# afermg/aliby

Measured on AMD Instinct MI355X. Metric: FOV tiles/sec (whole node), higher is better.
Workload: dtype u16 pixels, f64 feature accumulators, f32 dynamics, bfloat16 U-Net

## Files before the change

### aliby_amd/csrc/nn_conv.hip

```cpp
#include "common.h"
#include <utility>

typedef __bf16 bf16x8_t __attribute__((ext_vector_type(8)));
typedef float f32x16_t __attribute__((ext_vector_type(16)));
typedef float f32x2_t __attribute__((ext_vector_type(2)));

namespace {

template <class F, int... I>
__device__ __forceinline__ void static_for_impl(F&& f, std::integer_sequence<int, I...>) {
  (f(std::integral_constant<int, I>{}), ...);
}
template <int N, class F>
__device__ __forceinline__ void static_for(F&& f) {
  static_for_impl(static_cast<F&&>(f), std::make_integer_sequence<int, N>{});
}

__device__ __forceinline__ float cv_bf2f(unsigned h) { return __uint_as_float(h << 16); }
typedef __bf16 bf16x2_t __attribute__((ext_vector_type(2)));
__device__ __forceinline__ unsigned cv_pack2(float lo, float hi) {
  const f32x2_t f = {lo, hi};
  const bf16x2_t b = __builtin_convertvector(f, bf16x2_t);
  return __builtin_bit_cast(unsigned, b);
}
// ... 311 lines not shown
          const bool ok = lx != gapi && c >= 0 && c < a.W && !(bp == TW && kb == TW) && (unsigned)gy < (unsigned)a.H;
          const int img = (snd && ok) ? g0 + 1 : g0;
          inside |= (unsigned)ok << u;
          later |= (unsigned)snd << u;
          if constexpr (C3_HACK & 1) v[u] = make_uint4(cy, c, img, 3);
          else v[u] = inN[(unsigned)(((img * a.H + cy) * IW + min(max(c, 0), a.W - 1)) * a.cs + pl)];
        } else {
          const int gxi = x0 - 1 + lx;
          inside |= (unsigned)((unsigned)gy < (unsigned)a.H && (unsigned)gxi < (unsigned)a.W) << u;
          const int cx = min(max(gxi, 0), a.W - 1);
          if constexpr (C3_HACK & 1) v[u] = make_uint4(cy, cx, 2, 3);
          else v[u] = inN[(unsigned)(((UP ? cy >> 1 : cy) * IW + (UP ? cx >> 1 : cx)) * a.cs + pl)];
        }
      }
#pragma unroll
      for (int u = 0; u < BATCH; ++u) {
        if (it0 + u >= ITERS) break;
        uint4 o;
        if constexpr (PACK) {
          f32x2_t shs[4];
#pragma unroll
          for (int k = 0; k < 4; ++k) shs[k] = ((later >> u) & 1u) ? sh1[k] : sh[k];
          o = conv_act8(v[u], sc, shs, 0u - ((inside >> u) & 1u));
        } else {
          if constexpr (C3_HACK & 16) o = v[u]; else o = conv_act8(v[u], sc, sh, 0u - ((inside >> u) & 1u));
        }
        if (it0 + u == ITERS - 1 && p0 + (it0 + u) * PIX_PER_IT >= RAW) continue;
        if constexpr (C3_HACK & 32) { if (o.x == 0x12345u) lds[pl * PLANE + p0 + (it0 + u) * PIX_PER_IT] = o; }
        else lds[pl * PLANE + p0 + (it0 + u) * PIX_PER_IT] = o;
      }
    }
    if constexpr (PK > 0) {
      constexpr int POCT = 2 * PK, PUNITS = TH * TW * POCT;
      const uint4* pN = a.pin + (size_t)n * a.H * a.W * a.pcs;
#pragma unroll
      for (int it = 0; it < (PUNITS + 255) / 256; ++it) {
        const int u = tid + it * 256;
        if (u >= PUNITS) break;
        const int oct = u % POCT, pix = u / POCT;
        const int cy = min(y0 + pix / TW, a.H - 1), cx = min(x0 + pix % TW, a.W - 1);
        uint4 v = make_uint4(0, 0, 0, 0);
        if (oct < a.pcs) v = pN[(unsigned)((cy * a.W + cx) * a.pcs + oct)];
        ldsP[oct * PPLANE + pix] = v;
      }
    }
    CONV_STAMP(3);
    if constexpr (!(C3_HACK & 128)) __syncthreads();
    CONV_STAMP(4);

#pragma unroll
    for (int pass = 0; pass < PASSES; ++pass) {
      const int rbase = (rg * PASSES + pass) * R;
      f32x16_t acc[R];
      {
        float4 b4[4];
#pragma unroll
        for (int q = 0; q < 4; ++q) b4[q] = (C3_HACK & 64) ? make_float4(0.f, 0.f, 0.f, 0.f) : sbias[(c0 >> 2) + q];
        conv_seed<R>(acc, b4, rr, a.res != nullptr && !(C3_HACK & 2));
      }
      __builtin_amdgcn_sched_barrier(0);
      if (pass + 1 < PASSES && a.res && !(C3_HACK & 2)) load_res(pass + 1);
      __builtin_amdgcn_sched_barrier(0);
      if constexpr (!(C3_HACK & 8))
      conv_mfma<R, KC, (POOL ? cfg::DEPTH_POOL : cfg::DEPTH), PLANE, LW>(
          reinterpret_cast<const bf16x8_t*>(lds) + hh * PLANE + rbase * LW + px + second, wfrag, acc);
      if constexpr (PK > 0) {
        const bf16x8_t* LP = reinterpret_cast<const bf16x8_t*>(ldsP) + hh * PPLANE + rbase * TW + px;
#pragma unroll
        for (int r = 0; r < R; ++r)
#pragma unroll
          for (int k = 0; k < PK; ++k)
            acc[r] = __builtin_amdgcn_mfma_f32_32x32x16_bf16(pfrag[k], LP[2 * k * PPLANE + r * TW], acc[r], 0, 0, 0);
      }
      if (pass == PASSES - 1) CONV_STAMP(5);
      if constexpr (HEAD) {
        __builtin_amdgcn_sched_barrier(0);
#pragma unroll
        for (int r = 0; r < R; ++r) {
          const f32x16_t y = head_from_acc(acc[r], hconst, hconst + 32, hwf, hh);
          const int gy = y0 + rbase + r;
          if (hh == 0 && gx < a.W && gy < a.H) {
            float* hp = a.hout + (size_t)n * a.hO * a.H * a.W + (size_t)gy * a.W + gx;
            const float yo[4] = {y[0], y[1], y[2], y[3]};
            for (int o = 0; o < a.hO; ++o) hp[(size_t)o * a.H * a.W] = yo[o] + hconst[64 + o];
          }
        }
      }
      if ((!HEAD || a.out) && (!(C3_HACK & 4) || acc[0][3] == 12345.f)) conv_store<R>(a, nimg, irow, y0 + rbase, gx, c0, acc);
      if constexpr (POOL) {
        const int PH = a.H >> 1, PW = a.W >> 1;
#pragma unroll
        for (int r = 0; r < R; r += 2) {
          const int gy = y0 + rbase + r;
          const bool writer = (px & 1) == 0 && gx + 1 < a.W && gy + 1 < a.H;
          uint4* pp = a.pool + (size_t)nimg * PH * PW * a.ocs + a.ocoff + (unsigned)((((irow + gy) >> 1) * PW + (gx >> 1)) * a.ocs + (c0 >> 3));
#pragma unroll
          for (int half = 0; half < 2; ++half) {
            unsigned pk[4];
#pragma unroll
            for (int q = 0; q < 4; ++q) {
              const float v0 = fmaxf(acc[r][half * 8 + 2 * q], acc[r + 1][half * 8 + 2 * q]);
              const float v1 = fmaxf(acc[r][half * 8 + 2 * q + 1], acc[r + 1][half * 8 + 2 * q + 1]);
              pk[q] = cv_pack2(fmaxf(v0, __shfl_xor(v0, 1)), fmaxf(v1, __shfl_xor(v1, 1)));
            }
            if (writer) pp[half] = make_uint4(pk[0], pk[1], pk[2], pk[3]);
          }
        }
      }
    }
    CONV_STAMP(6);
  }
}

template <int CIN, int COUT, bool UP, bool PACK = false>
struct DmaCfg {
  static constexpr int KC = CIN / 16, NPL = CIN / 8, NCB = COUT / 32;
  static constexpr int WAVES_PER_SIMD = CIN >= 128 ? 1 : 2;
  static constexpr int R = CIN >= 64 ? 2 : 4;
  static constexpr int PASSES = (CIN >= 128 || COUT >= 128) ? 2 : 1;
  static constexpr int RG = 4 / NCB;
  static constexpr int TH = RG * R * PASSES, TW = 32, LH = TH + 2, LW = TW + 2 + (PACK ? 1 : 0);
  static constexpr int RAW = LH * LW;
  static constexpr int PLANE = NPL == 4 ? RAW + (10 - RAW % 8) % 8 : (RAW | 1);
  static constexpr int A_SLOTS = NPL * PLANE;
  static constexpr int PIX_PER_IT = 256 / NPL;
  static constexpr int ITERS = (RAW + PIX_PER_IT - 1) / PIX_PER_IT;
  static constexpr int RLH = UP ? TH / 2 + 2 : LH, RLW = UP ? TW / 2 + 2 : LW;
  static constexpr int RUNITS = RLH * RLW * NPL;
  static constexpr int GIT = (RUNITS + 255) / 256;
  static constexpr int R_SLOTS = GIT * 256;
  static constexpr int LDS_BYTES = (A_SLOTS + R_SLOTS) * 16;
  static constexpr int DEPTH = (CIN >= 64 && COUT >= 64) ? 4 : 6;
};

template <int CIN, int COUT, bool UP, bool PACK = false>
__global__ __launch_bounds__(256, (DmaCfg<CIN, COUT, UP, PACK>::WAVES_PER_SIMD)) void k_conv3x3_dma(ConvArgs a) {
  static_assert(!PACK || UP, "the packed LDS-DMA variant is written for upsampled input");
  using cfg = DmaCfg<CIN, COUT, UP, PACK>;
  constexpr int KC = cfg::KC, NPL = cfg::NPL, NCB = cfg::NCB, R = cfg::R, TH = cfg::TH, TW = cfg::TW;
  constexpr int LW = cfg::LW, RAW = cfg::RAW, PLANE = cfg::PLANE, RLW = cfg::RLW, PASSES = cfg::PASSES;
  constexpr int PIX_PER_IT = cfg::PIX_PER_IT, ITERS = cfg::ITERS, GIT = cfg::GIT;
  extern __shared__ uint4 lds[];
  uint4* const ldsA = lds;
  uint4* const ldsR = lds + cfg::A_SLOTS;

  const int tid = threadIdx.x, lane = tid & 63, wave = tid >> 6;
  const int cb = wave % NCB, rg = wave / NCB;
  const int px = lane & 31, hh = lane >> 5;
  const int c0 = cb * 32 + hh * 16;

  bf16x8_t wfrag[9 * KC];
  {
    const bf16x8_t* wp = reinterpret_cast<const bf16x8_t*>(a.wpk) + (size_t)cb * 9 * KC * 64 + lane;
#pragma unroll
    for (int i = 0; i < 9 * KC; ++i) wfrag[i] = wp[i * 64];
  }
  const int pl = tid % NPL, pix0 = tid / NPL;
  const int ly0 = pix0 / LW, lx0 = pix0 - ly0 * LW;
  f32x2_t sc[4];
#pragma unroll
  for (int k = 0; k < 4; ++k) sc[k] = f32x2_t{a.scale[pl * 8 + 2 * k], a.scale[pl * 8 + 2 * k + 1]};

  const int IH = UP ? a.H >> 1 : a.H, IW = UP ? a.W >> 1 : a.W;
  const int xcd = blockIdx.x & 7, slot = blockIdx.x >> 3, nslots = gridDim.x >> 3;
  const int per_xcd = (a.ntiles + 7) >> 3;
  const int t_end = min(a.ntiles, (xcd + 1) * per_xcd);
  const int wave_u = __builtin_amdgcn_readfirstlane(wave);

  auto issue_dma = [&](int tile) {
    const int tx = tile % a.tiles_x, tyn = tile / a.tiles_x;
    const int ty = tyn % a.tiles_y, n = tyn / a.tiles_y;
    const int ry0 = UP ? (ty * TH >> 1) - 1 : ty * TH - 1, rx0 = UP ? (tx * TW >> 1) - 1 : tx * TW - 1;
    int g0 = 0, cst = 0, half = 1 << 20;
    if constexpr (PACK) {
      g0 = (tx * TW) / a.W;
      cst = tx * TW - g0 * a.W;
      half = (a.W - cst) >> 1;
    }
    const uint4* inN = a.in + (size_t)(PACK ? n * a.G : n) * IH * IW * a.cs + a.coff;
    int t0 = tid;
    asm volatile("" : "+v"(t0));
#pragma unroll
    for (int k = 0; k < GIT; ++k) {
      const int unit = t0 + k * 256;
      const int rpix = unit / NPL, oct = unit % NPL;
      const int rly = rpix / RLW, rlx = rpix - rly * RLW;
      const int iy = min(max(ry0 + rly, 0), IH - 1);
      int ix, img = 0;
      if constexpr (PACK) {
        const bool first = rlx <= half;
        ix = min(max(first ? (cst >> 1) - 1 + rlx : rlx - half - 1, 0), IW - 1);
        img = first ? g0 : min(g0 + 1, a.G - 1);
      } else {
        ix = min(max(rx0 + rlx, 0), IW - 1);
      }
      const uint4* g = inN + (unsigned)(((img * IH + iy) * IW + ix) * a.cs + oct);
      __builtin_amdgcn_global_load_lds((const __attribute__((address_space(1))) void*)g,
                                       (__attribute__((address_space(3))) void*)(ldsR + k * 256 + wave_u * 64), 16, 0, 0);
    }
  };

  int tile = xcd * per_xcd + slot, stamp_tile = 0;
  if (tile < t_end) issue_dma(tile);
  for (; tile < t_end; tile += nslots, ++stamp_tile) {
    CONV_STAMP(0);
    const int tx = tile % a.tiles_x, tyn = tile / a.tiles_x;
    const int ty = tyn % a.tiles_y, n = tyn / a.tiles_y;
    const int y0 = ty * TH, x0 = tx * TW;
    int g0 = 0, cst = x0, kb = 1 << 20, nimg = n;
    if constexpr (PACK) {
      g0 = x0 / a.W;
      cst = x0 - g0 * a.W;
      kb = a.W - cst;
      nimg = n * a.G;
    }
    const int second = (PACK && px >= kb) ? 1 : 0;
    const int gx = PACK ? (second ? px - kb : cst + px) : x0 + px;
    const int irow = PACK ? (g0 + second) * a.H : 0;

    f32x2_t sh[4], sh1[PACK ? 4 : 1];
    {
      const float* sp = a.shift + (size_t)(nimg + g0) * a.shift_stride + pl * 8;
#pragma unroll
      for (int k = 0; k < 4; ++k) sh[k] = f32x2_t{sp[2 * k], sp[2 * k + 1]};
      if constexpr (PACK) {
        const float* sq = a.shift + (size_t)(nimg + min(g0 + 1, a.G - 1)) * a.shift_stride + pl * 8;
#pragma unroll
        for (int k = 0; k < 4; ++k) sh1[k] = f32x2_t{sq[2 * k], sq[2 * k + 1]};
      }
    }
    float4 b4[4] = {};
    if (a.bias) {
      const float4* bp = reinterpret_cast<const float4*>(a.bias + c0);
#pragma unroll
      for (int q = 0; q < 4; ++q) b4[q] = bp[q];
    }
    uint4 rr[R][2];
    auto load_res = [&](int pass) { conv_load_res<R>(a, nimg, irow, y0 + (rg * PASSES + pass) * R, gx, c0, rr); };
    if (a.res && !(C3_HACK & 2)) load_res(0);
    CONV_STAMP(1);
    asm volatile("s_waitcnt vmcnt(0)" ::: "memory");
    __syncthreads();
    CONV_STAMP(2);
    {
      const int ry0 = UP ? (y0 >> 1) - 1 : y0 - 1, rx0 = UP ? (x0 >> 1) - 1 : x0 - 1;
      int p0 = pix0, qy = ly0, qx = lx0;
      asm volatile("" : "+v"(p0), "+v"(qy), "+v"(qx));
#pragma unroll
      for (int it = 0; it < ITERS; ++it) {
        int lx = qx + (it * PIX_PER_IT) % LW, ly = qy + (it * PIX_PER_IT) / LW;
        if (lx >= LW) { lx -= LW; ly += 1; }
        const int gy = y0 - 1 + ly, gxi = x0 - 1 + lx;
        const int pix = p0 + it * PIX_PER_IT;
        unsigned keep;
        int rpix;
        uint4 o;
        if constexpr (PACK) {
          const int gapi = kb < 32 ? kb + 1 : TW + 2;
          const int bp = lx - 1 - (lx > gapi ? 1 : 0);
          const int snd = bp >= kb ? 1 : 0;
          const int c = snd ? bp - kb : cst + bp;
          keep = 0u - (unsigned)(lx != gapi && c >= 0 && c < a.W && !(bp == TW && kb == TW) && (unsigned)gy < (unsigned)a.H);
          const int rcol = snd ? (kb >> 1) + 1 + (c >> 1) : ((cst + bp) >> 1) - ((cst >> 1) - 1);
          rpix = min(max(((gy >> 1) - ry0) * RLW + rcol, 0), cfg::RLH * RLW - 1);
          f32x2_t shs[4];
#pragma unroll
          for (int k = 0; k < 4; ++k) shs[k] = snd ? sh1[k] : sh[k];
          o = conv_act8(ldsR[rpix * NPL + pl], sc, shs, keep);
        } else {
          keep = 0u - (unsigned)((unsigned)gy < (unsigned)a.H && (unsigned)gxi < (unsigned)a.W);
          rpix = UP ? min(((gy >> 1) - ry0) * RLW + ((gxi >> 1) - rx0), cfg::RLH * RLW - 1) : min(pix, RAW - 1);
          o = conv_act8(ldsR[rpix * NPL + pl], sc, sh, keep);
        }
        if (it == ITERS - 1 && pix >= RAW) continue;
        ldsA[pl * PLANE + pix] = o;
      }
    }
    CONV_STAMP(3);
    __syncthreads();
#pragma unroll
    for (int pass = 0; pass < PASSES; ++pass) {
      const int rbase = (rg * PASSES + pass) * R;
      f32x16_t acc[R];
      conv_seed<R>(acc, b4, rr, a.res != nullptr);
      __builtin_amdgcn_sched_barrier(0);
      if (pass == 0 && tile + nslots < t_end) issue_dma(tile + nslots);
      if (pass + 1 < PASSES && a.res) load_res(pass + 1);
      __builtin_amdgcn_sched_barrier(0);
      if (pass == 0) CONV_STAMP(4);
      conv_mfma<R, KC, cfg::DEPTH, PLANE, LW>(reinterpret_cast<const bf16x8_t*>(ldsA) + hh * PLANE + rbase * LW + px + second, wfrag, acc);
      if (pass == PASSES - 1) CONV_STAMP(5);
      conv_store<R>(a, nimg, irow, y0 + rbase, gx, c0, acc);
    }
    CONV_STAMP(6);
  }
}

struct PairCfg {
  static constexpr int KC = 2, NPL = 4, R = 2, PASSES = 2;
  static constexpr int TH = 14, TWO = 30, MH = 16, MW = 32, IH = 18, IW = 34;
  static constexpr int RAW_IN = IH * IW, PLANE_IN = RAW_IN + (10 - RAW_IN % 8) % 8;
  static constexpr int RAW_MID = MH * MW, PLANE_MID = RAW_MID + (10 - RAW_MID % 8) % 8;
  static constexpr int PIX_PER_IT = 256 / NPL, ITERS = (RAW_IN + PIX_PER_IT - 1) / PIX_PER_IT;
  static constexpr int MID_SLOTS = NPL * PLANE_MID + 8;
  static constexpr int SLOTS = NPL * PLANE_IN + 2 * MID_SLOTS;
  static constexpr int LDS_BYTES = SLOTS * 16;
  static constexpr int DEPTH = 6;
};

#ifndef CP_HACK
#define CP_HACK 0
#endif
template <bool POOL, bool HEAD>
__global__ __launch_bounds__(512, 1) void k_conv_pair32(ConvArgs a) {
  static_assert(!(POOL && HEAD), "either the pooled output (down block) or the output head (last unit)");
  using cfg = PairCfg;
  constexpr int KC = cfg::KC, NPL = cfg::NPL, R = cfg::R, PASSES = cfg::PASSES, TH = cfg::TH, TWO = cfg::TWO;
  constexpr int IW_ = cfg::IW, MW = cfg::MW, PLANE_IN = cfg::PLANE_IN, PLANE_MID = cfg::PLANE_MID, RAW_IN = cfg::RAW_IN;
  constexpr int PIX_PER_IT = cfg::PIX_PER_IT, ITERS = cfg::ITERS;
  extern __shared__ uint4 lds[];
  uint4* const ldsIn = lds;
  uint4* const ldsMid0 = lds + NPL * PLANE_IN;
  __shared__ __align__(16) float tabB[64];
  __shared__ float hconst[HEAD ? 2 * 32 + 4 : 1];

  const int consumer = threadIdx.x >> 8;
  const int tid = threadIdx.x & 255, lane = tid & 63, wave = tid >> 6;
  const int px = lane & 31, hh = lane >> 5;
  const int c0 = hh * 16;

  const int xcd = blockIdx.x & 7, slot = blockIdx.x >> 3, nslots = gridDim.x >> 3;
  const int per_xcd = (a.ntiles + 7) >> 3;
  const int t_begin = xcd * per_xcd + slot, t_end = min(a.ntiles, (xcd + 1) * per_xcd);
  const int my_tiles = t_begin < t_end ? (t_end - t_begin + nslots - 1) / nslots : 0;

  if (!consumer) {
    bf16x8_t wA[9 * KC];
    {
      const bf16x8_t* pa = reinterpret_cast<const bf16x8_t*>(a.wpk) + lane;
#pragma unroll
      for (int i = 0; i < 9 * KC; ++i) wA[i] = pa[i * 64];
    }
    const int pl = tid % NPL, pix0 = tid / NPL;
    const int ly0 = pix0 / IW_, lx0 = pix0 - ly0 * IW_;
    f32x2_t sc[4];
#pragma unroll
    for (int k = 0; k < 4; ++k) sc[k] = f32x2_t{a.scale[pl * 8 + 2 * k], a.scale[pl * 8 + 2 * k + 1]};
    uint4 v[ITERS];
    unsigned inside = 0;
    auto request = [&](int tile) {
      const int tx = tile % a.tiles_x, tyn = tile / a.tiles_x;
      const int ty = tyn % a.tiles_y, n = tyn / a.tiles_y;
      const int y0 = ty * TH, x0 = tx * TWO;
      const uint4* inN = a.in + (size_t)n * a.H * a.W * a.cs + a.coff;
      inside = 0;
#pragma unroll
      for (int u = 0; u < ITERS; ++u) {
        int lx = lx0 + (u * PIX_PER_IT) % IW_, ly = ly0 + (u * PIX_PER_IT) / IW_;
        if (lx >= IW_) { lx -= IW_; ly += 1; }
        const int gy = y0 - 2 + ly, gxi = x0 - 2 + lx;
        inside |= (unsigned)((unsigned)gy < (unsigned)a.H && (unsigned)gxi < (unsigned)a.W) << u;
        const int cy = min(max(gy, 0), a.H - 1), cx = min(max(gxi, 0), a.W - 1);
        if constexpr (CP_HACK & 1) v[u] = make_uint4(u, 1, 2, 3); else v[u] = inN[(unsigned)((cy * a.W + cx) * a.cs + pl)];
      }
    };
    if (my_tiles > 0) request(t_begin);
    for (int it = 0; it < my_tiles; ++it) {
      const int tile = t_begin + it * nslots;
      const int tx = tile % a.tiles_x, tyn = tile / a.tiles_x;
      const int ty = tyn % a.tiles_y, n = tyn / a.tiles_y;
      const int y0 = ty * TH, x0 = tx * TWO;
      uint4* const ldsMid = ldsMid0 + (it & 1) * cfg::MID_SLOTS;
      f32x2_t sh[4];
      {
        const float* sp = a.shift + (size_t)n * a.shift_stride + pl * 8;
#pragma unroll
        for (int k = 0; k < 4; ++k) sh[k] = f32x2_t{sp[2 * k], sp[2 * k + 1]};
      }
      if (tid < 32) {
        tabB[tid] = a.scale2[tid];
        tabB[32 + tid] = a.shift2[(size_t)n * a.shift2_stride + tid];
      }
#pragma unroll
      for (int u = 0; u < ITERS; ++u) {
        const uint4 o = conv_act8(v[u], sc, sh, 0u - ((inside >> u) & 1u));
        if (u == ITERS - 1 && pix0 + u * PIX_PER_IT >= RAW_IN) continue;
        if constexpr (!(CP_HACK & 64)) ldsIn[pl * PLANE_IN + pix0 + u * PIX_PER_IT] = o;
      }
      __syncthreads();
      if (it + 1 < my_tiles) request(tile + nslots);
      __builtin_amdgcn_sched_barrier(0);
#pragma unroll
      for (int pass = 0; pass < PASSES; ++pass) {
        const int mbase = (wave * PASSES + pass) * R;
        f32x16_t acc[R];
        {
          float4 b4[4] = {};
          if (a.bias) {
            const float4* bp = reinterpret_cast<const float4*>(a.bias + c0);
#pragma unroll
            for (int q = 0; q < 4; ++q) b4[q] = bp[q];
          }
#pragma unroll
          for (int r = 0; r < R; ++r)
#pragma unroll
            for (int q = 0; q < 4; ++q) { acc[r][4 * q] = b4[q].x; acc[r][4 * q + 1] = b4[q].y; acc[r][4 * q + 2] = b4[q].z; acc[r][4 * q + 3] = b4[q].w; }
        }
        __builtin_amdgcn_sched_barrier(0);
        if constexpr (!(CP_HACK & 8)) conv_mfma<R, KC, cfg::DEPTH, PLANE_IN, IW_>(reinterpret_cast<const bf16x8_t*>(ldsIn) + hh * PLANE_IN + mbase * IW_ + px, wA, acc);
        __builtin_amdgcn_sched_barrier(0);
        const int mgx = x0 - 1 + px;
#pragma unroll
        for (int r = 0; r < R; ++r) {
          const int mgy = y0 - 1 + mbase + r;
          const unsigned keep = 0u - (unsigned)((unsigned)mgy < (unsigned)a.H && (unsigned)mgx < (unsigned)a.W);
#pragma unroll
          for (int half = 0; half < 2; ++half) {
            f32x2_t s2[4], h2[4];
            const float4* tp = reinterpret_cast<const float4*>(tabB + c0 + 8 * half);
            const float4 sa = tp[0], sb = tp[1], ha = tp[8], hb = tp[9];
            s2[0] = f32x2_t{sa.x, sa.y}; s2[1] = f32x2_t{sa.z, sa.w}; s2[2] = f32x2_t{sb.x, sb.y}; s2[3] = f32x2_t{sb.z, sb.w};
            h2[0] = f32x2_t{ha.x, ha.y}; h2[1] = f32x2_t{ha.z, ha.w}; h2[2] = f32x2_t{hb.x, hb.y}; h2[3] = f32x2_t{hb.z, hb.w};
            const uint4 raw = make_uint4(cv_pack2(acc[r][8 * half + 0], acc[r][8 * half + 1]), cv_pack2(acc[r][8 * half + 2], acc[r][8 * half + 3]),
                                         cv_pack2(acc[r][8 * half + 4], acc[r][8 * half + 5]), cv_pack2(acc[r][8 * half + 6], acc[r][8 * half + 7]));
            if constexpr (!(CP_HACK & 32)) ldsMid[(2 * hh + half) * PLANE_MID + (mbase + r) * MW + px] = conv_act8(raw, s2, h2, keep);
          }
        }
      }
      __syncthreads();
    }
    __syncthreads();
    __syncthreads();
  } else {
    bf16x8_t wB[9 * KC];
    {
      const bf16x8_t* pb = reinterpret_cast<const bf16x8_t*>(a.wpk2) + lane;
#pragma unroll
      for (int i = 0; i < 9 * KC; ++i) wB[i] = pb[i * 64];
    }
    HeadW hwf;
    if constexpr (HEAD) {
      hwf = head_weights(a.hw, a.hO, lane);
      if (tid < 32) {
        hconst[tid] = a.hscale[tid];
        hconst[32 + tid] = a.hshift[tid];
        if (tid < 4) hconst[64 + tid] = tid < a.hO ? a.hbias[tid] : 0.f;
      }
    }
    float4 b4[4] = {};
    if (a.bias2) {
      const float4* bp = reinterpret_cast<const float4*>(a.bias2 + c0);
#pragma unroll
      for (int q = 0; q < 4; ++q) b4[q] = bp[q];
    }
    __syncthreads();
    __syncthreads();
    for (int it = 0; it < my_tiles; ++it) {
      const int tile = t_begin + it * nslots;
      const int tx = tile % a.tiles_x, tyn = tile / a.tiles_x;
      const int ty = tyn % a.tiles_y, n = tyn / a.tiles_y;
      const int y0 = ty * TH, x0 = tx * TWO;
      const uint4* const ldsMid = ldsMid0 + (it & 1) * cfg::MID_SLOTS;
      const int gx = (px < TWO && x0 + px < a.W) ? x0 + px : a.W;
#pragma unroll
      for (int pass = 0; pass < PASSES; ++pass) {
        const int rbase = (wave * PASSES + pass) * R;
        if (rbase < TH) {
          uint4 rr[R][2];
          if (a.res && !(CP_HACK & 2)) conv_load_res<R>(a, n, 0, y0 + rbase, min(gx, a.W - 1), c0, rr);
          f32x16_t acc[R];
          conv_seed<R>(acc, b4, rr, a.res != nullptr && !(CP_HACK & 2));
          __builtin_amdgcn_sched_barrier(0);
          if constexpr (!(CP_HACK & 16)) conv_mfma<R, KC, cfg::DEPTH, PLANE_MID, MW>(reinterpret_cast<const bf16x8_t*>(ldsMid) + hh * PLANE_MID + rbase * MW + px, wB, acc);
          if constexpr (HEAD) {
#pragma unroll
            for (int r = 0; r < R; ++r) {
              const f32x16_t y = head_from_acc(acc[r], hconst, hconst + 32, hwf, hh);
              const int gy = y0 + rbase + r;
              if (hh == 0 && gx < a.W && gy < a.H) {
                float* hp = a.hout + (size_t)n * a.hO * a.H * a.W + (size_t)gy * a.W + gx;
                const float yo[4] = {y[0], y[1], y[2], y[3]};
                for (int o = 0; o < a.hO; ++o) hp[(size_t)o * a.H * a.W] = yo[o] + hconst[64 + o];
              }
            }
          }
          if ((!HEAD || a.out) && (!(CP_HACK & 4) || acc[0][3] == 12345.f)) conv_store<R>(a, n, 0, y0 + rbase, gx, c0, acc);
          if constexpr (POOL) {
            const int PH = a.H >> 1, PW = a.W >> 1;
            const int gy = y0 + rbase;
            const bool writer = (px & 1) == 0 && gx + 1 < a.W && gy + 1 < a.H;
            uint4* pp = a.pool + (size_t)n * PH * PW * a.ocs + a.ocoff + (unsigned)(((gy >> 1) * PW + (min(gx, a.W - 1) >> 1)) * a.ocs + (c0 >> 3));
#pragma unroll
            for (int half = 0; half < 2; ++half) {
              unsigned pk[4];
#pragma unroll
              for (int q = 0; q < 4; ++q) {
                const float v0 = fmaxf(acc[0][half * 8 + 2 * q], acc[1][half * 8 + 2 * q]);
                const float v1 = fmaxf(acc[0][half * 8 + 2 * q + 1], acc[1][half * 8 + 2 * q + 1]);
                pk[q] = cv_pack2(fmaxf(v0, __shfl_xor(v0, 1)), fmaxf(v1, __shfl_xor(v1, 1)));
              }
              if (writer && (!(CP_HACK & 4) || acc[0][3] == 12345.f)) pp[half] = make_uint4(pk[0], pk[1], pk[2], pk[3]);
            }
          }
        }
        __syncthreads();
      }
    }
  }
}

struct FirstPairCfg {
  static constexpr int KC = 2, NPL = 4, R = 2, PASSES = 2;
  static constexpr int TH = 14, TWO = 30, MH = 16, MW = 32, AH = 18, AW = 36;
  static constexpr int RAW_MID = MH * MW, PLANE_MID = RAW_MID + (10 - RAW_MID % 8) % 8;
  static constexpr int MID_SLOTS = NPL * PLANE_MID + 8;
  static constexpr int P0_WORDS = 2 * AH * AW;
  static constexpr int RAWP_WORDS = MH * MW;
  static constexpr int VALS = 2 * AH * AW, ITERS = (VALS + 255) / 256;
  static constexpr int LDS_BYTES = 2 * MID_SLOTS * 16 + P0_WORDS * 4 + 2 * RAWP_WORDS * 4;
  static constexpr int DEPTH = 6;
};

__global__ __launch_bounds__(512, 1) void k_conv_first_pair(ConvArgs a) {
  using cfg = FirstPairCfg;
  constexpr int KC = cfg::KC, R = cfg::R, PASSES = cfg::PASSES, TH = cfg::TH, TWO = cfg::TWO, MW = cfg::MW;
  constexpr int AH = cfg::AH, AW = cfg::AW, PLANE_MID = cfg::PLANE_MID, ITERS = cfg::ITERS;
  extern __shared__ uint4 lds[];
  uint4* const ldsMid0 = lds;
  unsigned* const P0 = reinterpret_cast<unsigned*>(lds + 2 * cfg::MID_SLOTS);
  unsigned* const rawP0 = P0 + cfg::P0_WORDS;
  __shared__ __align__(16) float tabB[64];

  const int consumer = threadIdx.x >> 8;
  const int tid = threadIdx.x & 255, lane = tid & 63, wave = tid >> 6;
  const int px = lane & 31, hh = lane >> 5;
  const int c0 = hh * 16;

  const int xcd = blockIdx.x & 7, slot = blockIdx.x >> 3, nslots = gridDim.x >> 3;
  const int per_xcd = (a.ntiles + 7) >> 3;
  const int t_begin = xcd * per_xcd + slot, t_end = min(a.ntiles, (xcd + 1) * per_xcd);
  const int my_tiles = t_begin < t_end ? (t_end - t_begin + nslots - 1) / nslots : 0;
  const size_t plane = (size_t)a.H * a.W;

  if (!consumer) {
    bf16x8_t wF[2];
    {
      const int m = lane & 31, co = 16 * ((m >> 2) & 1) + (m & 3) + 4 * (m >> 3);
#pragma unroll
      for (int kc = 0; kc < 2; ++kc) {
        unsigned r4[4];
#pragma unroll
        for (int j2 = 0; j2 < 4; ++j2) {
          float v[2];
#pragma unroll
          for (int e = 0; e < 2; ++e) {
            const int k = 16 * kc + 8 * hh + 2 * j2 + e, c = k / 12, ty = (k % 12) / 4, tx = k % 4;
            v[e] = (c < a.fcin && tx < 3 && k < 24) ? a.fw[((size_t)co * a.fcin + c) * 9 + ty * 3 + tx] : 0.f;
          }
          r4[j2] = cv_pack2(v[0], v[1]);
        }
        wF[kc] = __builtin_bit_cast(bf16x8_t, make_uint4(r4[0], r4[1], r4[2], r4[3]));
      }
    }
    int goff[2][2];
    unsigned gmask[2][2];
#pragma unroll
    for (int kc = 0; kc < 2; ++kc)
#pragma unroll
      for (int g = 0; g < 2; ++g) {
        const int k = 16 * kc + 8 * hh + 4 * g;
        const bool live = k < 24 && k / 12 < a.fcin;
        goff[kc][g] = live ? (k / 12) * AH * AW + ((k % 12) / 4) * AW : 0;
        gmask[kc][g] = live ? 0xffffffffu : 0u;
      }
    if (tid < 32) {
      tabB[tid] = a.scale2[tid];
      tabB[32 + tid] = a.shift2[tid];
    }
    const float fs0 = a.fscale[0], fh0 = a.fshift[0];
    const float fs1 = a.fcin > 1 ? a.fscale[1] : 0.f, fh1 = a.fcin > 1 ? a.fshift[1] : 0.f;
    float v[ITERS];
    unsigned inside = 0;
    auto request = [&](int tile) {
      const int tx = tile % a.tiles_x, tyn = tile / a.tiles_x;
      const int ty = tyn % a.tiles_y, n = tyn / a.tiles_y;
      const int y0 = ty * TH, x0 = tx * TWO;
      inside = 0;
#pragma unroll
      for (int u = 0; u < ITERS; ++u) {
        const int i = tid + 256 * u;
        const int c = i / (AH * AW), rem = i - c * (AH * AW), r = rem / AW, q = rem - r * AW;
        const int gy = y0 - 2 + r, gx = x0 - 2 + q;
        const bool ok = i < cfg::VALS && c < a.fcin && (unsigned)gy < (unsigned)a.H && (unsigned)gx < (unsigned)a.W;
        inside |= (unsigned)ok << u;
        const int cy = min(max(gy, 0), a.H - 1), cx = min(max(gx, 0), a.W - 1), cc = min(c, a.fcin - 1);
        v[u] = a.fx[((size_t)n * a.fcin + cc) * plane + (size_t)cy * a.W + cx];
      }
    };
    if (my_tiles > 0) request(t_begin);
    unsigned short* const P0h = reinterpret_cast<unsigned short*>(P0);
    for (int it = 0; it < my_tiles; ++it) {
      const int tile = t_begin + it * nslots;
      const int tx = tile % a.tiles_x, tyn = tile / a.tiles_x;
      const int ty = tyn % a.tiles_y;
      const int y0 = ty * TH, x0 = tx * TWO;
      uint4* const ldsMid = ldsMid0 + (it & 1) * cfg::MID_SLOTS;
      unsigned short* const rawPh = reinterpret_cast<unsigned short*>(rawP0 + (it & 1) * cfg::RAWP_WORDS);
#pragma unroll
      for (int u = 0; u < ITERS; ++u) {
        const int i = tid + 256 * u;
        if (i >= cfg::VALS) break;
        const int c = i / (AH * AW), rem = i - c * (AH * AW), r = rem / AW, q = rem - r * AW;
        const bool ok = (inside >> u) & 1u;
        const float t = ok ? fmaxf(v[u] * (c ? fs1 : fs0) + (c ? fh1 : fh0), 0.f) : 0.f;
        const unsigned short b = (unsigned short)(cv_pack2(t, 0.f) & 0xffffu);
        P0h[2 * i] = b;
        if (q > 0) P0h[2 * (i - 1) + 1] = b;
        if (q == AW - 1) P0h[2 * i + 1] = 0;
        if (r >= 2 && q >= 2 && q < 2 + MW)
          rawPh[2 * ((r - 2) * MW + (q - 2)) + c] = (unsigned short)(cv_pack2(ok ? v[u] : 0.f, 0.f) & 0xffffu);
      }
      if (a.fcin < 2) {
        for (int i = tid; i < cfg::RAWP_WORDS; i += 256) rawPh[2 * i + 1] = 0;
      }
      __syncthreads();
      if (it + 1 < my_tiles) request(tile + nslots);
      __builtin_amdgcn_sched_barrier(0);
#pragma unroll
      for (int pass = 0; pass < PASSES; ++pass) {
        const int mbase = (wave * PASSES + pass) * R;
        const int mgx = x0 - 1 + px;
#pragma unroll
        for (int r = 0; r < R; ++r) {
          const int m = mbase + r;
          f32x16_t acc;
#pragma unroll
          for (int k = 0; k < 16; ++k) acc[k] = 0.f;
#pragma unroll
          for (int kc = 0; kc < 2; ++kc) {
            const unsigned* w0 = P0 + goff[kc][0] + m * AW + px;
            const unsigned* w1 = P0 + goff[kc][1] + m * AW + px;
            const uint4 bfrag = make_uint4(w0[0] & gmask[kc][0], w0[2] & gmask[kc][0], w1[0] & gmask[kc][1], w1[2] & gmask[kc][1]);
            acc = __builtin_amdgcn_mfma_f32_32x32x16_bf16(wF[kc], __builtin_bit_cast(bf16x8_t, bfrag), acc, 0, 0, 0);
          }
          const int mgy = y0 - 1 + m;
          const unsigned keep = 0u - (unsigned)((unsigned)mgy < (unsigned)a.H && (unsigned)mgx < (unsigned)a.W);
#pragma unroll
          for (int half = 0; half < 2; ++half) {
            f32x2_t s2[4], h2[4];
            const float4* tp = reinterpret_cast<const float4*>(tabB + c0 + 8 * half);
            const float4 sa = tp[0], sb = tp[1], ha = tp[8], hb = tp[9];
            s2[0] = f32x2_t{sa.x, sa.y}; s2[1] = f32x2_t{sa.z, sa.w}; s2[2] = f32x2_t{sb.x, sb.y}; s2[3] = f32x2_t{sb.z, sb.w};
            h2[0] = f32x2_t{ha.x, ha.y}; h2[1] = f32x2_t{ha.z, ha.w}; h2[2] = f32x2_t{hb.x, hb.y}; h2[3] = f32x2_t{hb.z, hb.w};
            const uint4 raw = make_uint4(cv_pack2(acc[8 * half + 0], acc[8 * half + 1]), cv_pack2(acc[8 * half + 2], acc[8 * half + 3]),
                                         cv_pack2(acc[8 * half + 4], acc[8 * half + 5]), cv_pack2(acc[8 * half + 6], acc[8 * half + 7]));
            ldsMid[(2 * hh + half) * PLANE_MID + m * MW + px] = conv_act8(raw, s2, h2, keep);
          }
        }
      }
      __syncthreads();
    }
    __syncthreads();
    __syncthreads();
  } else {
    bf16x8_t wB[9 * KC];
    {
      const bf16x8_t* pb = reinterpret_cast<const bf16x8_t*>(a.wpk2) + lane;
#pragma unroll
      for (int i = 0; i < 9 * KC; ++i) wB[i] = pb[i * 64];
    }
    const bf16x8_t pfrag = (reinterpret_cast<const bf16x8_t*>(a.pwpk) + lane)[0];
    float4 b4[4] = {};
    if (a.bias2) {
      const float4* bp = reinterpret_cast<const float4*>(a.bias2 + c0);
#pragma unroll
      for (int q = 0; q < 4; ++q) b4[q] = bp[q];
    }
    __syncthreads();
    __syncthreads();
    for (int it = 0; it < my_tiles; ++it) {
      const int tile = t_begin + it * nslots;
      const int tx = tile % a.tiles_x, tyn = tile / a.tiles_x;
      const int ty = tyn % a.tiles_y, n = tyn / a.tiles_y;
      const int y0 = ty * TH, x0 = tx * TWO;
      const uint4* const ldsMid = ldsMid0 + (it & 1) * cfg::MID_SLOTS;
      const unsigned* const rawP = rawP0 + (it & 1) * cfg::RAWP_WORDS;
      const int gx = (px < TWO && x0 + px < a.W) ? x0 + px : a.W;
#pragma unroll
      for (int pass = 0; pass < PASSES; ++pass) {
        const int rbase = (wave * PASSES + pass) * R;
        if (rbase < TH) {
          f32x16_t acc[R];
#pragma unroll
          for (int r = 0; r < R; ++r)
#pragma unroll
            for (int q = 0; q < 4; ++q) { acc[r][4 * q] = b4[q].x; acc[r][4 * q + 1] = b4[q].y; acc[r][4 * q + 2] = b4[q].z; acc[r][4 * q + 3] = b4[q].w; }
          __builtin_amdgcn_sched_barrier(0);
          conv_mfma<R, KC, cfg::DEPTH, PLANE_MID, MW>(reinterpret_cast<const bf16x8_t*>(ldsMid) + hh * PLANE_MID + rbase * MW + px, wB, acc);
#pragma unroll
          for (int r = 0; r < R; ++r) {
            const unsigned w = hh ? 0u : rawP[(rbase + r) * MW + px];
            acc[r] = __builtin_amdgcn_mfma_f32_32x32x16_bf16(pfrag, __builtin_bit_cast(bf16x8_t, make_uint4(w, 0u, 0u, 0u)), acc[r], 0, 0, 0);
          }
          conv_store<R>(a, n, 0, y0 + rbase, gx, c0, acc);
        }
        __syncthreads();
      }
    }
  }
}

__global__ __launch_bounds__(256) void k_out_head_mfma(const uint4* __restrict__ x, const float* __restrict__ scale, const float* __restrict__ shift,
                                                       const float* __restrict__ w, const float* __restrict__ bias, int O, size_t N, size_t P,
                                                       float* __restrict__ out) {
  __shared__ float hconst[2 * 32 + 4];
  const int tid = threadIdx.x, lane = tid & 63, px = lane & 31, hh = lane >> 5;
  if (tid < 32) {
    hconst[tid] = scale[tid];
    hconst[32 + tid] = shift[tid];
    if (tid < 4) hconst[64 + tid] = tid < O ? bias[tid] : 0.f;
  }
  const HeadW hwf = head_weights(w, O, lane);
  __syncthreads();
  const size_t total = N * P, nblk = (total + 31) / 32;
  const size_t wave0 = ((size_t)blockIdx.x * blockDim.x + tid) >> 6, nwaves = ((size_t)gridDim.x * blockDim.x) >> 6;
  for (size_t b = wave0; b < nblk; b += nwaves) {
    const size_t pix = b * 32 + px;
    const bool ok = pix < total;
    const size_t q = ok ? pix : total - 1;
    const uint4 lo = x[q * 4 + 2 * hh], hi = x[q * 4 + 2 * hh + 1];
    const f32x16_t y = head_apply(lo, hi, hconst, hconst + 32, hwf, hh);
    if (ok && hh == 0) {
      const size_t n = pix / P, p = pix - n * P;
      const float yo[4] = {y[0], y[1], y[2], y[3]};
      for (int o = 0; o < O; ++o) out[(n * O + o) * P + p] = yo[o] + hconst[64 + o];
    }
  }
}

__global__ void k_pack_conv3x3(const float* w, int cout, int cin_src, int cin, int taps, unsigned short* out, size_t total) {
  const size_t i = (size_t)blockIdx.x * blockDim.x + threadIdx.x;
  if (i >= total) return;
  const int j = (int)(i & 7), lane = (int)((i >> 3) & 63);
  size_t rest = i >> 9;
  const int kcn = cin / 16;
  const int kc = (int)(rest % kcn);
  rest /= kcn;
  const int tap = (int)(rest % taps), cb = (int)(rest / taps);
  const int m = lane & 31, h = lane >> 5;
  const int co = cb * 32 + 16 * ((m >> 2) & 1) + (m & 3) + 4 * (m >> 3);
  const int ci = 16 * kc + 8 * h + j;
  float v = 0.f;
  if (ci < cin_src && co < cout) v = w[((size_t)co * cin_src + ci) * taps + tap];
  out[i] = (unsigned short)cv_f2bf(v);
}

unsigned long long* g_conv_trace = nullptr;

template <int CIN, int COUT, bool UP, bool PACK = false>
int launch_conv_dma(aliby_ctx* ctx, ConvArgs& a, hipStream_t stream) {
  using cfg = DmaCfg<CIN, COUT, UP, PACK>;
  a.G = PACK ? 224 / a.W : 1;
  a.tiles_x = PACK ? 224 / cfg::TW : (a.W + cfg::TW - 1) / cfg::TW;
  a.tiles_y = (a.H + cfg::TH - 1) / cfg::TH;
  const long long nt = (long long)(a.N / a.G) * a.tiles_x * a.tiles_y;
  ARG_CHECK(nt < INT_MAX, "conv3x3: too many tiles");
  a.ntiles = (int)nt;
  static bool attr_done = false;
  if (!attr_done) {
    HIP_TRY(hipFuncSetAttribute(reinterpret_cast<const void*>(&k_conv3x3_dma<CIN, COUT, UP, PACK>),
                                hipFuncAttributeMaxDynamicSharedMemorySize, cfg::LDS_BYTES));
    attr_done = true;
  }
  const int per_xcd = (a.ntiles + 7) / 8;
  const int cap = 32 * cfg::WAVES_PER_SIMD;
  const int nslots = per_xcd < cap ? per_xcd : cap;
  hipLaunchKernelGGL((k_conv3x3_dma<CIN, COUT, UP, PACK>), dim3(8 * nslots), dim3(256), cfg::LDS_BYTES, stream, a);
  KERNEL_CHECK();
  return ALIBY_OK;
}

template <int CIN, int COUT, bool UP, bool TALL, bool PACK = false>
int launch_conv_reg(aliby_ctx* ctx, ConvArgs& a, hipStream_t stream) {
  using cfg = ConvCfg<CIN, COUT, TALL, PACK>;
  a.G = PACK ? 224 / a.W : 1;
  a.tiles_x = PACK ? 224 / cfg::TW : (a.W + cfg::TW - 1) / cfg::TW;
  a.tiles_y = (a.H + cfg::TH - 1) / cfg::TH;
  const long long nt = (long long)(a.N / a.G) * a.tiles_x * a.tiles_y;
  ARG_CHECK(nt < INT_MAX, "conv3x3: too many tiles");
  a.ntiles = (int)nt;
  static bool attr_done = false;
  constexpr int PKV = PACK ? 0 : (!UP && CIN == 32 && COUT == 32) ? 1 : ((!UP && CIN == 64 && COUT == 64) ? 2 : 0);
  constexpr int P_BYTES = PKV ? 2 * PKV * ((cfg::TH * cfg::TW) | 1) * 16 : 0;
  if (!attr_done) {
    HIP_TRY(hipFuncSetAttribute(reinterpret_cast<const void*>(&k_conv3x3<CIN, COUT, UP, false, 0, TALL, PACK>),
                                hipFuncAttributeMaxDynamicSharedMemorySize, cfg::LDS_BYTES));
    HIP_TRY(hipFuncSetAttribute(reinterpret_cast<const void*>(&k_conv3x3<CIN, COUT, UP, true, 0, TALL, PACK>),
                                hipFuncAttributeMaxDynamicSharedMemorySize, cfg::LDS_BYTES));
    if constexpr (PKV > 0)
      HIP_TRY(hipFuncSetAttribute(reinterpret_cast<const void*>(&k_conv3x3<CIN, COUT, UP, false, PKV, TALL>),
                                  hipFuncAttributeMaxDynamicSharedMemorySize, cfg::LDS_BYTES + P_BYTES));
    attr_done = true;
  }
  const int per_xcd = (a.ntiles + 7) / 8;
  const int nslots = per_xcd < 64 ? per_xcd : 64;
  if (a.pin) {
    if constexpr (PKV > 0) {
      ARG_CHECK(!a.pool && a.pcs >= 1 && a.pcs <= 2 * PKV, "conv3x3: fused projection: unsupported input width");
// ... 264 lines not shown
```

Baseline: 592.5.

## Double-buffer input window and prefetch residuals in paired conv kernel

The producer half of the fused conv pair kernel now keeps two LDS input windows and two scale/shift tables. This lets it stage tile it+1 and issue global loads for tile it+2 while consumers work on tile it. The consumer half now prefetches residual rows for the next tile into registers before its MFMA work, and it cuts its barriers from one per pass to one per tile. In exchange the kernel uses more LDS and more registers, and the producer/consumer barrier pairing is reordered, which carries a risk of mismatched sync.

```diff
diff --git a/aliby_amd/csrc/nn_conv.hip b/aliby_amd/csrc/nn_conv.hip
--- a/aliby_amd/csrc/nn_conv.hip
+++ b/aliby_amd/csrc/nn_conv.hip
@@ -637,10 +637,13 @@
   static constexpr int RAW_IN = IH * IW, PLANE_IN = RAW_IN + (10 - RAW_IN % 8) % 8;
   static constexpr int RAW_MID = MH * MW, PLANE_MID = RAW_MID + (10 - RAW_MID % 8) % 8;
   static constexpr int PIX_PER_IT = 256 / NPL, ITERS = (RAW_IN + PIX_PER_IT - 1) / PIX_PER_IT;
+  static constexpr int IN_SLOTS = NPL * PLANE_IN;
   static constexpr int MID_SLOTS = NPL * PLANE_MID + 8;
-  static constexpr int SLOTS = NPL * PLANE_IN + 2 * MID_SLOTS;
+  static constexpr int SLOTS = 2 * IN_SLOTS + 2 * MID_SLOTS;
   static constexpr int LDS_BYTES = SLOTS * 16;
   static constexpr int DEPTH = 6;
+  static_assert(IN_SLOTS % 8 == 0, "window buffers must start on an 8-slot boundary");
+  static_assert(LDS_BYTES + 2 * 64 * 4 + (2 * 32 + 4) * 4 <= 160 * 1024, "one workgroup per CU");
 };
 
 #ifndef CP_HACK
@@ -654,9 +657,9 @@
   constexpr int IW_ = cfg::IW, MW = cfg::MW, PLANE_IN = cfg::PLANE_IN, PLANE_MID = cfg::PLANE_MID, RAW_IN = cfg::RAW_IN;
   constexpr int PIX_PER_IT = cfg::PIX_PER_IT, ITERS = cfg::ITERS;
   extern __shared__ uint4 lds[];
-  uint4* const ldsIn = lds;
-  uint4* const ldsMid0 = lds + NPL * PLANE_IN;
-  __shared__ __align__(16) float tabB[64];
+  uint4* const ldsIn0 = lds;
+  uint4* const ldsMid0 = lds + 2 * cfg::IN_SLOTS;
+  __shared__ __align__(16) float tabB[2][64];
   __shared__ float hconst[HEAD ? 2 * 32 + 4 : 1];
 
   const int consumer = threadIdx.x >> 8;
@@ -683,7 +686,8 @@
     for (int k = 0; k < 4; ++k) sc[k] = f32x2_t{a.scale[pl * 8 + 2 * k], a.scale[pl * 8 + 2 * k + 1]};
     uint4 v[ITERS];
     unsigned inside = 0;
-    auto request = [&](int tile) {
+    auto request = [&](int it) {
+      const int tile = t_begin + it * nslots;
       const int tx = tile % a.tiles_x, tyn = tile / a.tiles_x;
       const int ty = tyn % a.tiles_y, n = tyn / a.tiles_y;
       const int y0 = ty * TH, x0 = tx * TWO;
@@ -699,13 +703,10 @@
         if constexpr (CP_HACK & 1) v[u] = make_uint4(u, 1, 2, 3); else v[u] = inN[(unsigned)((cy * a.W + cx) * a.cs + pl)];
       }
     };
-    if (my_tiles > 0) request(t_begin);
-    for (int it = 0; it < my_tiles; ++it) {
+    auto stage = [&](int it) {
       const int tile = t_begin + it * nslots;
-      const int tx = tile % a.tiles_x, tyn = tile / a.tiles_x;
-      const int ty = tyn % a.tiles_y, n = tyn / a.tiles_y;
-      const int y0 = ty * TH, x0 = tx * TWO;
-      uint4* const ldsMid = ldsMid0 + (it & 1) * cfg::MID_SLOTS;
+      const int n = tile / a.tiles_x / a.tiles_y;
+      uint4* const ldsIn = ldsIn0 + (it & 1) * cfg::IN_SLOTS;
       f32x2_t sh[4];
       {
         const float* sp = a.shift + (size_t)n * a.shift_stride + pl * 8;
@@ -713,8 +714,8 @@
         for (int k = 0; k < 4; ++k) sh[k] = f32x2_t{sp[2 * k], sp[2 * k + 1]};
       }
       if (tid < 32) {
-        tabB[tid] = a.scale2[tid];
-        tabB[32 + tid] = a.shift2[(size_t)n * a.shift2_stride + tid];
+        tabB[it & 1][tid] = a.scale2[tid];
+        tabB[it & 1][32 + tid] = a.shift2[(size_t)n * a.shift2_stride + tid];
       }
 #pragma unroll
       for (int u = 0; u < ITERS; ++u) {
@@ -722,9 +723,21 @@
         if (u == ITERS - 1 && pix0 + u * PIX_PER_IT >= RAW_IN) continue;
         if constexpr (!(CP_HACK & 64)) ldsIn[pl * PLANE_IN + pix0 + u * PIX_PER_IT] = o;
       }
-      __syncthreads();
-      if (it + 1 < my_tiles) request(tile + nslots);
-      __builtin_amdgcn_sched_barrier(0);
+    };
+    if (my_tiles > 0) {
+      request(0);
+      stage(0);
+      if (my_tiles > 1) request(1);
+    }
+    __syncthreads();
+    for (int it = 0; it < my_tiles; ++it) {
+      const int tile = t_begin + it * nslots;
+      const int tx = tile % a.tiles_x, tyn = tile / a.tiles_x;
+      const int ty = tyn % a.tiles_y;
+      const int y0 = ty * TH, x0 = tx * TWO;
+      const uint4* const ldsIn = ldsIn0 + (it & 1) * cfg::IN_SLOTS;
+      uint4* const ldsMid = ldsMid0 + (it & 1) * cfg::MID_SLOTS;
+      const float* const tab = tabB[it & 1];
 #pragma unroll
       for (int pass = 0; pass < PASSES; ++pass) {
         const int mbase = (wave * PASSES + pass) * R;
@@ -752,7 +765,7 @@
 #pragma unroll
           for (int half = 0; half < 2; ++half) {
             f32x2_t s2[4], h2[4];
-            const float4* tp = reinterpret_cast<const float4*>(tabB + c0 + 8 * half);
+            const float4* tp = reinterpret_cast<const float4*>(tab + c0 + 8 * half);
             const float4 sa = tp[0], sb = tp[1], ha = tp[8], hb = tp[9];
             s2[0] = f32x2_t{sa.x, sa.y}; s2[1] = f32x2_t{sa.z, sa.w}; s2[2] = f32x2_t{sb.x, sb.y}; s2[3] = f32x2_t{sb.z, sb.w};
             h2[0] = f32x2_t{ha.x, ha.y}; h2[1] = f32x2_t{ha.z, ha.w}; h2[2] = f32x2_t{hb.x, hb.y}; h2[3] = f32x2_t{hb.z, hb.w};
@@ -762,10 +775,13 @@
           }
         }
       }
+      __builtin_amdgcn_sched_barrier(0);
+      if (it + 1 < my_tiles) {
+        stage(it + 1);
+        if (it + 2 < my_tiles) request(it + 2);
+      }
       __syncthreads();
     }
-    __syncthreads();
-    __syncthreads();
   } else {
     bf16x8_t wB[9 * KC];
     {
@@ -788,7 +804,21 @@
 #pragma unroll
       for (int q = 0; q < 4; ++q) b4[q] = bp[q];
     }
-    __syncthreads();
+    const bool has_res = a.res != nullptr && !(CP_HACK & 2);
+    uint4 rr[PASSES][R][2];
+    auto request_res = [&](int it, int pass) {
+      const int tile = t_begin + it * nslots;
+      const int tx = tile % a.tiles_x, tyn = tile / a.tiles_x;
+      const int ty = tyn % a.tiles_y, n = tyn / a.tiles_y;
+      const int x0 = tx * TWO;
+      const int gx = (px < TWO && x0 + px < a.W) ? x0 + px : a.W - 1;
+      conv_load_res<R>(a, n, 0, ty * TH + (wave * PASSES + pass) * R, gx, c0, rr[pass]);
+    };
+    if (has_res && my_tiles > 0) {
+#pragma unroll
+      for (int pass = 0; pass < PASSES; ++pass)
+        if ((wave * PASSES + pass) * R < TH) request_res(0, pass);
+    }
     __syncthreads();
     for (int it = 0; it < my_tiles; ++it) {
       const int tile = t_begin + it * nslots;
@@ -797,14 +827,14 @@
       const int y0 = ty * TH, x0 = tx * TWO;
       const uint4* const ldsMid = ldsMid0 + (it & 1) * cfg::MID_SLOTS;
       const int gx = (px < TWO && x0 + px < a.W) ? x0 + px : a.W;
+      __syncthreads();
 #pragma unroll
       for (int pass = 0; pass < PASSES; ++pass) {
         const int rbase = (wave * PASSES + pass) * R;
         if (rbase < TH) {
-          uint4 rr[R][2];
-          if (a.res && !(CP_HACK & 2)) conv_load_res<R>(a, n, 0, y0 + rbase, min(gx, a.W - 1), c0, rr);
           f32x16_t acc[R];
-          conv_seed<R>(acc, b4, rr, a.res != nullptr && !(CP_HACK & 2));
+          conv_seed<R>(acc, b4, rr[pass], has_res);
+          if (has_res && it + 1 < my_tiles) request_res(it + 1, pass);
           __builtin_amdgcn_sched_barrier(0);
           if constexpr (!(CP_HACK & 16)) conv_mfma<R, KC, cfg::DEPTH, PLANE_MID, MW>(reinterpret_cast<const bf16x8_t*>(ldsMid) + hh * PLANE_MID + rbase * MW + px, wB, acc);
           if constexpr (HEAD) {
@@ -838,7 +868,6 @@
             }
           }
         }
-        __syncthreads();
       }
     }
   }
```

After: 594.8 (median of 6 runs). About the same (+0.4%).
